# jizongFox/MI-based-Regularized-Semi-supervised-Segmentation

Hardware: AMD Instinct MI355X
Metric: images/sec (UNet+IIC fwd/bwd) ACDC 256^2 (higher is better)
Workload: dtype bf16; 1 GPU; udaiic train step, ACDC-shaped 1x256x256 4-class slices, LB=UB=16 per GPU, taps Conv5/Up_conv3/Up_conv2, K=20 x 5 sub-heads, paddings [1,3] (BASELINE configs[1]); mi_precision=f16f8, global_batch=32, parallelism=dp1, launch_tape=True, tape_ops=170, tape_replays_in_run=449

## Files before the change

mi-based-regularized-semi-supervised-segmentation_amd/csrc/api.hip:

```cpp
#include <stdarg.h>

#include "common.h"

namespace miseg_core {
static thread_local char g_err[512] = "";
char* last_error_buf() { return g_err; }
int fail(int code, const char* fmt, ...) {
    va_list ap;
    va_start(ap, fmt);
    vsnprintf(g_err, sizeof(g_err), fmt, ap);
    va_end(ap);
    return code;
}
}

extern "C" int miseg_version(void) { return 418; }
extern "C" const char* miseg_last_error(void) { return miseg::last_error_buf(); }

namespace miseg_core {
static hipEvent_t next_fork_event() {
    constexpr int kRing = 256, kDev = 16;
    struct Ring { hipEvent_t ev[kRing]; int made = 0, next = 0; };
    static thread_local Ring rings[kDev];
    int dev = 0;
    if (hipGetDevice(&dev) != hipSuccess || dev < 0 || dev >= kDev) return nullptr;
    Ring& r = rings[dev];
    constexpr unsigned flags = hipEventDisableTiming | hipEventDisableSystemFence;
    if (r.made < kRing) {
        if (hipEventCreateWithFlags(&r.ev[r.made], flags) != hipSuccess) return nullptr;
        ++r.made;
    }
    hipEvent_t ev = r.ev[r.next % r.made];
    r.next = (r.next + 1) % kRing;
    return ev;
}
}

extern "C" int miseg_stream_wait_stream(void* waiter, void* producer) {
    MISEG_TAPE(miseg_stream_wait_stream, waiter, producer);
    if (waiter == producer) return MISEG_OK;
    hipEvent_t ev = miseg_core::next_fork_event();
    if (!ev) return miseg_core::fail(MISEG_E_LAUNCH, "stream_wait_stream: hipEventCreateWithFlags failed");
    hipError_t e = hipEventRecord(ev, reinterpret_cast<hipStream_t>(producer));
    if (e == hipSuccess) e = hipStreamWaitEvent(reinterpret_cast<hipStream_t>(waiter), ev, 0);
    if (e != hipSuccess) return miseg_core::fail(MISEG_E_LAUNCH, "stream_wait_stream: %s", hipGetErrorString(e));
    return MISEG_OK;
}
```

mi-based-regularized-semi-supervised-segmentation_amd/csrc/conv_wgrad.hip:

```cpp
#include "conv.h"

namespace miseg {

constexpr int WG_TH = 8, WG_TW = 32, WG_P = 34;

template <typename T, bool BNL = false>
__global__ __launch_bounds__(kCT, 1) void conv3x3_wgrad_kernel(ConvSrc src, int N, int H, int W, const T* __restrict__ gout, int Cout,
                                                              int nsplit, float* __restrict__ partials, BnLoad bl) {
    extern __shared__ __attribute__((aligned(16))) float wsm[];
    float* Gs = wsm;
    float* Is = wsm + WG_TH * WG_TW * WG_P;
    const int Cin = src.C0 + src.C1;
    const int tid = threadIdx.x, lane = tid & 63, wv = tid >> 6, l15 = lane & 15, kq = lane >> 4;
    const int split = blockIdx.x, ci0 = blockIdx.y * 32, co0 = blockIdx.z * 32;
    const int tilesC = (W + WG_TW - 1) / WG_TW, tilesR = (H + WG_TH - 1) / WG_TH;
    const int ntiles = N * tilesR * tilesC;
    constexpr int IW = WG_TW + 2;
    f32x4 acc[2][18];
#pragma unroll
    for (int a = 0; a < 2; ++a)
#pragma unroll
        for (int b = 0; b < 18; ++b) acc[a][b] = f32x4{0.f, 0.f, 0.f, 0.f};
    float bc[kBwdCoefRows] = {0.f, 0.f, 0.f, 0.f, 0.f, 0.f};
    if (BNL && co0 + (tid & 31) < Cout)
#pragma unroll
        for (int r = 0; r < kBwdCoefRows; ++r) bc[r] = bl.coef[(size_t)r * Cout + co0 + (tid & 31)];

    for (int tile = split; tile < ntiles; tile += nsplit) {
        const int tc = tile % tilesC, tr = (tile / tilesC) % tilesR, n = tile / (tilesC * tilesR);
        const int h0 = tr * WG_TH, w0 = tc * WG_TW;
        __syncthreads();
        for (int idx = tid; idx < WG_TH * WG_TW * 32; idx += kCT) {
            const int c = idx & 31, px = idx >> 5, ix = px % WG_TW, iy = px / WG_TW;
            const int h = h0 + iy, w = w0 + ix;
            float v = 0.f;
            if (h < H && w < W && co0 + c < Cout) {
                const size_t o = (((size_t)n * H + h) * W + w) * Cout + co0 + c;
                v = to_f32(gout[o]);
                if (BNL) {
                    const float g = to_f32(reinterpret_cast<const T*>(bl.gy)[o]);
                    const float lin = bc[4] + bc[5] * (v - bc[2]);
                    v = v * bc[0] + bc[1] > relu_keep_threshold<T>() ? bc[3] * g + lin : lin;
                }
            }
            Gs[px * WG_P + c] = v;
        }
        for (int idx = tid; idx < (WG_TH + 2) * IW * 32; idx += kCT) {
            const int c = idx & 31, px = idx >> 5, ix = px % IW, iy = px / IW;
            const int h = h0 - 1 + iy, w = w0 - 1 + ix, cc = ci0 + c;
            float v = 0.f;
            if (h >= 0 && h < H && w >= 0 && w < W && cc < Cin) {
                if (cc < src.C0) {
                    const int hs = H >> src.ups0, wsz = W >> src.ups0;
                    v = to_f32(reinterpret_cast<const T*>(src.p0)[(((size_t)n * hs + (h >> src.ups0)) * wsz + (w >> src.ups0)) * src.C0 + cc]);
                } else {
                    const int hs = H >> src.ups1, wsz = W >> src.ups1;
                    v = to_f32(reinterpret_cast<const T*>(src.p1)[(((size_t)n * hs + (h >> src.ups1)) * wsz + (w >> src.ups1)) * src.C1 + cc - src.C0]);
                }
            }
            Is[px * WG_P + c] = v;
        }
        __syncthreads();
#pragma unroll 1
        for (int rr = 0; rr < 2; ++rr) {
            const int row = wv * 2 + rr;
#pragma unroll 1
            for (int cs = 0; cs < WG_TW; cs += 4) {
                const float a0 = Gs[(row * WG_TW + cs + kq) * WG_P + l15];
                const float a1 = Gs[(row * WG_TW + cs + kq) * WG_P + 16 + l15];
#pragma unroll
                for (int tap = 0; tap < 9; ++tap) {
                    const int ky = tap / 3, kx = tap % 3;
                    const float* ip = Is + ((row + ky) * IW + cs + kq + kx) * WG_P + l15;
                    const float b0 = ip[0], b1 = ip[16];
                    acc[0][tap * 2 + 0] = __builtin_amdgcn_mfma_f32_16x16x4f32(a0, b0, acc[0][tap * 2 + 0], 0, 0, 0);
                    acc[0][tap * 2 + 1] = __builtin_amdgcn_mfma_f32_16x16x4f32(a0, b1, acc[0][tap * 2 + 1], 0, 0, 0);
                    acc[1][tap * 2 + 0] = __builtin_amdgcn_mfma_f32_16x16x4f32(a1, b0, acc[1][tap * 2 + 0], 0, 0, 0);
                    acc[1][tap * 2 + 1] = __builtin_amdgcn_mfma_f32_16x16x4f32(a1, b1, acc[1][tap * 2 + 1], 0, 0, 0);
                }
            }
        }
    }
    float* Ds = wsm;
    for (int w = 0; w < 4; ++w) {
        __syncthreads();
        if (wv == w) {
#pragma unroll
            for (int a = 0; a < 2; ++a)
#pragma unroll
                for (int b = 0; b < 18; ++b)
#pragma unroll
                    for (int r = 0; r < 4; ++r) {
                        const int co = a * 16 + kq * 4 + r, col = (b / 2) * 32 + (b % 2) * 16 + l15;
                        if (w == 0) Ds[co * 288 + col] = acc[a][b][r];
                        else Ds[co * 288 + col] += acc[a][b][r];
                    }
        }
    }
    __syncthreads();
    float* outp = partials + (((size_t)split * gridDim.z + blockIdx.z) * gridDim.y + blockIdx.y) * (32 * 288);
    for (int e = tid; e < 32 * 288; e += kCT) outp[e] = Ds[e];
}

typedef __bf16 bf16x8_t __attribute__((ext_vector_type(8)));
typedef float f32x16 __attribute__((ext_vector_type(16)));
#define LDS_S16X4(ptr) ((__attribute__((address_space(3))) s16x4*)(ptr))

__device__ __forceinline__ bf16x8_t tr_frag32(const short* row_px0, int kq, int q, int p) {
    s16x4 lo = __builtin_amdgcn_ds_read_tr16_b64_v4i16(LDS_S16X4(row_px0 + (4 * kq + q) * 16 + 4 * p));
    s16x4 hi = __builtin_amdgcn_ds_read_tr16_b64_v4i16(LDS_S16X4(row_px0 + (16 + 4 * kq + q) * 16 + 4 * p));
    s16x8 f = {lo[0], lo[1], lo[2], lo[3], hi[0], hi[1], hi[2], hi[3]};
    return __builtin_bit_cast(bf16x8_t, f);
}

__device__ __forceinline__ bf16x8_t tr_frag(const short* blk_px0, int q, int p) {
    s16x4 lo = __builtin_amdgcn_ds_read_tr16_b64_v4i16(LDS_S16X4(blk_px0 + q * 16 + 4 * p));
    s16x4 hi = __builtin_amdgcn_ds_read_tr16_b64_v4i16(LDS_S16X4(blk_px0 + (4 + q) * 16 + 4 * p));
    s16x8 f = {lo[0], lo[1], lo[2], lo[3], hi[0], hi[1], hi[2], hi[3]};
    return __builtin_bit_cast(bf16x8_t, f);
}

template <bool BNL>
__global__ __launch_bounds__(kCT, 2) void conv3x3_wgrad_bf16_kernel(ConvSrc src, int N, int H, int W, const bf16* __restrict__ gout,
                                                                   int Cout, int nsplit, float* __restrict__ partials, BnLoad bl) {
    constexpr int IW = WG_TW + 2, NPX = WG_TH * WG_TW, NIPX = (WG_TH + 2) * IW;
    extern __shared__ __attribute__((aligned(16))) unsigned char wsm_raw[];
    constexpr int GSUB = NPX * 16 + 64;
    short* Gs = reinterpret_cast<short*>(wsm_raw);
    short* Is = Gs + 2 * GSUB;
    static_assert((NIPX * 32) % 256 == 128, "Is sub-tiles: re-check the bank offset for this tile shape");
    const int Cin = src.C0 + src.C1;
    const int tid = threadIdx.x, lane = tid & 63, wv = tid >> 6, l15 = lane & 15, kq = lane >> 4;
    const int g8 = 8 * kq, q = (lane >> 2) & 3, p4 = lane & 3;
    const int split = blockIdx.x, ci0 = blockIdx.y * 32, co0 = blockIdx.z * 32;
    const int tilesC = (W + WG_TW - 1) / WG_TW, tilesR = (H + WG_TH - 1) / WG_TH;
    const int ntiles = N * tilesR * tilesC;
    f32x16 acc[3];
#pragma unroll
    for (int b = 0; b < 3; ++b)
#pragma unroll
        for (int r = 0; r < 16; ++r) acc[b][r] = 0.f;
    const int wvu = __builtin_amdgcn_readfirstlane(wv);
    const int tap0 = 2 * wvu, tap1 = 2 * wvu + 1;
    const int off0 = ((tap0 / 3) * IW + tap0 % 3) * 16, off1 = ((tap1 / 3) * IW + tap1 % 3) * 16, off8 = (2 * IW + 2) * 16;
    const uint4 zero4 = make_uint4(0, 0, 0, 0);
    const int g16 = lane >> 4, chh = g16 & 1, pxh = g16 >> 1;

    constexpr int NG = NPX * 4 / kCT, NI = (NIPX * 4 + kCT - 1) / kCT;
    uint4 pg[NG], pi[NI];
    uint4 pr[BNL ? NG : 1];
    unsigned okg = 0;
    float* Cf = reinterpret_cast<float*>(Is + 2 * NIPX * 16);
    if (BNL) {
        for (int idx = tid; idx < kBwdCoefRows * 32; idx += kCT) Cf[idx] = co0 + (idx & 31) < Cout ? bl.coef[(size_t)(idx >> 5) * Cout + co0 + (idx & 31)] : 0.f;
        __syncthreads();
    }
    int g_iy[NG], g_ix[NG], g_rel[NG];
    int i_iy[NI], i_ix[NI], i_rel[NI], i_src[NI];
    {
        const int hs0 = H >> src.ups0, ws0 = W >> src.ups0, ws1 = W >> src.ups1;
        (void)hs0;
#pragma unroll
        for (int j = 0; j < NG; ++j) {
            const int idx = tid + kCT * j, v = idx & 3, px = idx >> 2, c = co0 + v * 8;
            g_ix[j] = px % WG_TW, g_iy[j] = px / WG_TW;
            g_rel[j] = c < Cout ? (g_iy[j] * W + g_ix[j]) * Cout + c : -1;
        }
#pragma unroll
        for (int j = 0; j < NI; ++j) {
            const int idx = tid + kCT * j, v = idx & 3, px = idx >> 2, cc = ci0 + v * 8;
            i_ix[j] = px % IW - 1, i_iy[j] = px / IW - 1;
            const bool slot = idx < NIPX * (3 + 1) && cc < Cin, first = cc < src.C0;
            i_src[j] = slot ? (first ? 0 : 1) : -1;
            i_rel[j] = first ? ((i_iy[j] >> src.ups0) * ws0 + (i_ix[j] >> src.ups0)) * src.C0 + cc
                             : ((i_iy[j] >> src.ups1) * ws1 + (i_ix[j] >> src.ups1)) * src.C1 + cc - src.C0;
        }
    }
    auto fetch = [&](int tile) __attribute__((always_inline)) {
        const int tc = tile % tilesC, tr = (tile / tilesC) % tilesR, n = tile / (tilesC * tilesR);
        const int h0 = tr * WG_TH, w0 = tc * WG_TW;
        const bf16* gcorner = gout + (((size_t)n * H + h0) * W + w0) * Cout;
        const bf16* ycorner = BNL ? reinterpret_cast<const bf16*>(bl.gy) + (((size_t)n * H + h0) * W + w0) * Cout : nullptr;
        const bf16* s0 = reinterpret_cast<const bf16*>(src.p0) + (((size_t)n * (H >> src.ups0) + (h0 >> src.ups0)) * (W >> src.ups0) + (w0 >> src.ups0)) * src.C0;
        const bf16* s1 = reinterpret_cast<const bf16*>(src.p1) + (((size_t)n * (H >> src.ups1) + (h0 >> src.ups1)) * (W >> src.ups1) + (w0 >> src.ups1)) * src.C1;
        okg = 0;
#pragma unroll
        for (int j = 0; j < NG; ++j) {
            uint4 val = zero4;
            if (g_rel[j] >= 0 && g_iy[j] < H - h0 && g_ix[j] < W - w0) {
                if (BNL) { pr[j] = *reinterpret_cast<const uint4*>(gcorner + g_rel[j]); val = *reinterpret_cast<const uint4*>(ycorner + g_rel[j]); okg |= 1u << j; }
                else val = *reinterpret_cast<const uint4*>(gcorner + g_rel[j]);
            }
            pg[j] = val;
        }
#pragma unroll
        for (int j = 0; j < NI; ++j) {
            uint4 val = zero4;
            if (i_src[j] >= 0 && (unsigned)(h0 + i_iy[j]) < (unsigned)H && (unsigned)(w0 + i_ix[j]) < (unsigned)W)
                val = *reinterpret_cast<const uint4*>((i_src[j] ? s1 : s0) + i_rel[j]);
            pi[j] = val;
        }
    };
    if (split < ntiles) fetch(split);
    for (int tile = split; tile < ntiles; tile += nsplit) {
        __syncthreads();
        if (BNL) {
            asm volatile("" ::: "memory");
            float cf[kBwdCoefRows][8];
#pragma unroll
            for (int r = 0; r < kBwdCoefRows; ++r)
#pragma unroll
                for (int i = 0; i < 8; i += 4) {
                    const float4 q = *reinterpret_cast<const float4*>(Cf + r * 32 + (tid & 3) * 8 + i);
                    cf[r][i] = q.x; cf[r][i + 1] = q.y; cf[r][i + 2] = q.z; cf[r][i + 3] = q.w;
                }
#pragma unroll
            for (int j = 0; j < NG; ++j)
                pg[j] = (okg >> j) & 1u ? bn_graw_vec<bf16>(pr[j], pg[j], cf[0], cf[1], cf[2], cf[3], cf[4], cf[5]) : zero4;
        }
#pragma unroll
        for (int j = 0; j < NG; ++j) {
            const int idx = tid + kCT * j, v = idx & 3, px = idx >> 2;
            *reinterpret_cast<uint4*>(Gs + (v >> 1) * GSUB + px * 16 + (v & 1) * 8) = pg[j];
        }
#pragma unroll
        for (int j = 0; j < NI; ++j) {
            const int idx = tid + kCT * j, v = idx & 3, px = idx >> 2;
            if (idx < NIPX * 4) *reinterpret_cast<uint4*>(Is + ((v >> 1) * NIPX + px) * 16 + (v & 1) * 8) = pi[j];
        }
        __syncthreads();
        if (tile + nsplit < ntiles) fetch(tile + nsplit);
#pragma unroll 2
        for (int row = 0; row < WG_TH; ++row) {
            const short* gb = Gs + chh * GSUB + (row * WG_TW + 8 * pxh) * 16;
            const bf16x8_t a0 = tr_frag(gb, q, p4), a1 = tr_frag(gb + 16 * 16, q, p4);
            const short* ib = Is + (chh * NIPX + row * IW + 8 * pxh) * 16;
            {
                const bf16x8_t b0 = tr_frag(ib + off0, q, p4), b1 = tr_frag(ib + off0 + 16 * 16, q, p4);
                acc[0] = __builtin_amdgcn_mfma_f32_32x32x16_bf16(a0, b0, acc[0], 0, 0, 0);
                acc[0] = __builtin_amdgcn_mfma_f32_32x32x16_bf16(a1, b1, acc[0], 0, 0, 0);
            }
            {
                const bf16x8_t b0 = tr_frag(ib + off1, q, p4), b1 = tr_frag(ib + off1 + 16 * 16, q, p4);
                acc[1] = __builtin_amdgcn_mfma_f32_32x32x16_bf16(a0, b0, acc[1], 0, 0, 0);
                acc[1] = __builtin_amdgcn_mfma_f32_32x32x16_bf16(a1, b1, acc[1], 0, 0, 0);
            }
            if ((row >> 1) == wvu) {
                const bf16x8_t b0 = tr_frag(ib + off8, q, p4), b1 = tr_frag(ib + off8 + 16 * 16, q, p4);
                acc[2] = __builtin_amdgcn_mfma_f32_32x32x16_bf16(a0, b0, acc[2], 0, 0, 0);
                acc[2] = __builtin_amdgcn_mfma_f32_32x32x16_bf16(a1, b1, acc[2], 0, 0, 0);
            }
        }
    }
    float* Ds = reinterpret_cast<float*>(wsm_raw);
    float* D8 = Ds + 32 * 288;
    __syncthreads();
#pragma unroll
    for (int r = 0; r < 16; ++r) {
        const int co = (r & 3) + 8 * (r >> 2) + 4 * (lane >> 5), ci = lane & 31;
        Ds[co * 288 + tap0 * 32 + ci] = acc[0][r];
        Ds[co * 288 + tap1 * 32 + ci] = acc[1][r];
        D8[wvu * 1024 + co * 32 + ci] = acc[2][r];
    }
    __syncthreads();
    float* outp = partials + (((size_t)split * gridDim.z + blockIdx.z) * gridDim.y + blockIdx.y) * (32 * 288);
    for (int e = tid; e < 32 * 288; e += kCT) {
        const int co = e / 288, col = e - co * 288;
        float v = Ds[e];
        if (col >= 256) {
            const int i8 = co * 32 + col - 256;
            v = (D8[i8] + D8[1024 + i8]) + (D8[2048 + i8] + D8[3072 + i8]);
        }
        outp[e] = v;
    }
}

template <bool BNL>
__global__ __launch_bounds__(kCT, BNL ? 3 : 4) void conv3x3_wgrad_bf16_c16_kernel(ConvSrc src, int N, int H, int W, const bf16* __restrict__ gout,
                                                                       int Cout, int nsplit, float* __restrict__ partials, BnLoad bl) {
    constexpr int IW = WG_TW + 2, NPX = WG_TH * WG_TW, NIPX = (WG_TH + 2) * IW;
    extern __shared__ __attribute__((aligned(16))) unsigned char wsm_raw[];
    short* Gs = reinterpret_cast<short*>(wsm_raw);
    short* Is = Gs + NPX * 16;
    const int Cin = src.C0 + src.C1;
    const int tid = threadIdx.x, lane = tid & 63, wv = tid >> 6, l15 = lane & 15, kq = lane >> 4;
    const int q = (lane >> 2) & 3, p4 = lane & 3;
    const int split = blockIdx.x, ci0 = blockIdx.y * 16, co0 = blockIdx.z * 16;
    const int tilesC = (W + WG_TW - 1) / WG_TW, tilesR = (H + WG_TH - 1) / WG_TH;
    const int ntiles = N * tilesR * tilesC;
    f32x4 acc[9];
#pragma unroll
    for (int b = 0; b < 9; ++b) acc[b] = f32x4{0.f, 0.f, 0.f, 0.f};
    const uint4 zero4 = make_uint4(0, 0, 0, 0);
    constexpr int NG = NPX * 2 / kCT, NI = (NIPX * 2 + kCT - 1) / kCT;
    uint4 pg[NG], pi[NI];
    uint4 pr[BNL ? NG : 1];
    unsigned okg = 0;
    float* Cf = reinterpret_cast<float*>(Is + NIPX * 16);
    if (BNL) {
        for (int idx = tid; idx < kBwdCoefRows * 16; idx += kCT) Cf[idx] = co0 + (idx & 15) < Cout ? bl.coef[(size_t)(idx >> 4) * Cout + co0 + (idx & 15)] : 0.f;
        __syncthreads();
    }
    int g_iy[NG], g_ix[NG], g_rel[NG];
    int i_iy[NI], i_ix[NI], i_rel[NI], i_src[NI];
    {
        const int hs0 = H >> src.ups0, ws0 = W >> src.ups0, ws1 = W >> src.ups1;
        (void)hs0;
#pragma unroll
        for (int j = 0; j < NG; ++j) {
            const int idx = tid + kCT * j, v = idx & 1, px = idx >> 1, c = co0 + v * 8;
            g_ix[j] = px % WG_TW, g_iy[j] = px / WG_TW;
            g_rel[j] = c < Cout ? (g_iy[j] * W + g_ix[j]) * Cout + c : -1;
        }
#pragma unroll
        for (int j = 0; j < NI; ++j) {
            const int idx = tid + kCT * j, v = idx & 1, px = idx >> 1, cc = ci0 + v * 8;
            i_ix[j] = px % IW - 1, i_iy[j] = px / IW - 1;
            const bool slot = idx < NIPX * (1 + 1) && cc < Cin, first = cc < src.C0;
            i_src[j] = slot ? (first ? 0 : 1) : -1;
            i_rel[j] = first ? ((i_iy[j] >> src.ups0) * ws0 + (i_ix[j] >> src.ups0)) * src.C0 + cc
                             : ((i_iy[j] >> src.ups1) * ws1 + (i_ix[j] >> src.ups1)) * src.C1 + cc - src.C0;
        }
    }
    auto fetch = [&](int tile) __attribute__((always_inline)) {
        const int tc = tile % tilesC, tr = (tile / tilesC) % tilesR, n = tile / (tilesC * tilesR);
        const int h0 = tr * WG_TH, w0 = tc * WG_TW;
        const bf16* gcorner = gout + (((size_t)n * H + h0) * W + w0) * Cout;
        const bf16* ycorner = BNL ? reinterpret_cast<const bf16*>(bl.gy) + (((size_t)n * H + h0) * W + w0) * Cout : nullptr;
        const bf16* s0 = reinterpret_cast<const bf16*>(src.p0) + (((size_t)n * (H >> src.ups0) + (h0 >> src.ups0)) * (W >> src.ups0) + (w0 >> src.ups0)) * src.C0;
        const bf16* s1 = reinterpret_cast<const bf16*>(src.p1) + (((size_t)n * (H >> src.ups1) + (h0 >> src.ups1)) * (W >> src.ups1) + (w0 >> src.ups1)) * src.C1;
        okg = 0;
#pragma unroll
        for (int j = 0; j < NG; ++j) {
            uint4 val = zero4;
            if (g_rel[j] >= 0 && g_iy[j] < H - h0 && g_ix[j] < W - w0) {
                if (BNL) { pr[j] = *reinterpret_cast<const uint4*>(gcorner + g_rel[j]); val = *reinterpret_cast<const uint4*>(ycorner + g_rel[j]); okg |= 1u << j; }
                else val = *reinterpret_cast<const uint4*>(gcorner + g_rel[j]);
            }
            pg[j] = val;
        }
#pragma unroll
        for (int j = 0; j < NI; ++j) {
            uint4 val = zero4;
            if (i_src[j] >= 0 && (unsigned)(h0 + i_iy[j]) < (unsigned)H && (unsigned)(w0 + i_ix[j]) < (unsigned)W)
                val = *reinterpret_cast<const uint4*>((i_src[j] ? s1 : s0) + i_rel[j]);
            pi[j] = val;
        }
    };
    if (split < ntiles) fetch(split);
    for (int tile = split; tile < ntiles; tile += nsplit) {
        __syncthreads();
        if (BNL) {
            asm volatile("" ::: "memory");
            float cf[kBwdCoefRows][8];
#pragma unroll
            for (int r = 0; r < kBwdCoefRows; ++r)
#pragma unroll
                for (int i = 0; i < 8; i += 4) {
                    const float4 q = *reinterpret_cast<const float4*>(Cf + r * 16 + (tid & 1) * 8 + i);
                    cf[r][i] = q.x; cf[r][i + 1] = q.y; cf[r][i + 2] = q.z; cf[r][i + 3] = q.w;
                }
#pragma unroll
            for (int j = 0; j < NG; ++j)
                pg[j] = (okg >> j) & 1u ? bn_graw_vec<bf16>(pr[j], pg[j], cf[0], cf[1], cf[2], cf[3], cf[4], cf[5]) : zero4;
        }
#pragma unroll
        for (int j = 0; j < NG; ++j) {
            const int idx = tid + kCT * j;
            *reinterpret_cast<uint4*>(Gs + (idx >> 1) * 16 + (idx & 1) * 8) = pg[j];
        }
#pragma unroll
        for (int j = 0; j < NI; ++j) {
            const int idx = tid + kCT * j;
            if (idx < NIPX * 2) *reinterpret_cast<uint4*>(Is + (idx >> 1) * 16 + (idx & 1) * 8) = pi[j];
        }
        __syncthreads();
        if (tile + nsplit < ntiles) fetch(tile + nsplit);
#pragma unroll
        for (int rr = 0; rr < 2; ++rr) {
            const int row = wv * 2 + rr;
            const bf16x8_t a0 = tr_frag32(Gs + row * WG_TW * 16, kq, q, p4);
#pragma unroll
            for (int tap = 0; tap < 9; ++tap) {
                const int ky = tap / 3, kx = tap % 3;
                const bf16x8_t b0 = tr_frag32(Is + ((row + ky) * IW + kx) * 16, kq, q, p4);
                acc[tap] = __builtin_amdgcn_mfma_f32_16x16x32_bf16(a0, b0, acc[tap], 0, 0, 0);
            }
        }
    }
    float* Ds = reinterpret_cast<float*>(wsm_raw);
    for (int w = 0; w < 4; ++w) {
        __syncthreads();
        if (wv == w) {
#pragma unroll
            for (int tap = 0; tap < 9; ++tap)
#pragma unroll
                for (int r = 0; r < 4; ++r) {
                    const int o = (kq * 4 + r) * 144 + tap * 16 + l15;
                    if (w == 0) Ds[o] = acc[tap][r];
                    else Ds[o] += acc[tap][r];
                }
        }
    }
    __syncthreads();
    const int nci32 = (Cin + 31) / 32, nco32 = (Cout + 31) / 32;
    float* outp = partials + (((size_t)split * nco32 + blockIdx.z / 2) * nci32 + blockIdx.y / 2) * (32 * 288) + (blockIdx.y & 1) * 16;
    for (int e = tid; e < 16 * 144; e += kCT) {
        const int co = (blockIdx.z & 1) * 16 + e / 144, tap = (e % 144) / 16, ci = e % 16;
        outp[co * 288 + tap * 32 + ci] = Ds[e];
    }
}

__global__ __launch_bounds__(256) void wgrad_reduce_kernel(const float* __restrict__ partials, int nsplit, int Cout, int Cin, int nco,
                                                           int nci, float* __restrict__ gw) {
    const size_t stride = (size_t)nco * nci * (32 * 288);
    reduce_partials_block(partials, nsplit, stride, nco * nci * 32 * 288, gw, [](int e) { return (size_t)e; }, [=](int e) {
        const int ci32 = e & 31, tap = (e >> 5) % 9, co32 = (e / 288) & 31, tile = e / (32 * 288);
        const int co = (tile / nci) * 32 + co32, ci = (tile % nci) * 32 + ci32;
        return (co < Cout && ci < Cin) ? (co * Cin + ci) * 9 + tap : -1;
    });
}

}

using namespace miseg;

namespace miseg {
__global__ __launch_bounds__(256) void slice_cin_kernel(const float* __restrict__ src, int Cout, int Cin_pad, int Cin, float* __restrict__ dst) {
    const int total = Cout * Cin * 9;
    for (int e = blockIdx.x * 256 + threadIdx.x; e < total; e += gridDim.x * 256) {
        const int t = e % 9, ci = (e / 9) % Cin, co = e / (9 * Cin);
        dst[e] = src[((size_t)co * Cin_pad + ci) * 9 + t];
    }
}
}
extern "C" int miseg_conv3x3_wgrad_slice(void* stream, const float* gw_padded, int64_t Cout, int64_t Cin_pad, int64_t Cin, float* gw) {
    MISEG_TAPE(miseg_conv3x3_wgrad_slice, stream, gw_padded, Cout, Cin_pad, Cin, gw);
    MISEG_REQUIRE(gw_padded && gw && Cout > 0 && Cin > 0 && Cin <= Cin_pad, "conv3x3_wgrad_slice: bad args");
    const int total = (int)(Cout * Cin * 9);
    hipLaunchKernelGGL(slice_cin_kernel, dim3(std::min((total + 255) / 256, 256)), dim3(256), 0, as_stream(stream), gw_padded, (int)Cout, (int)Cin_pad,
                       (int)Cin, gw);
    MISEG_LAUNCH_CHECK("slice_cin_kernel");
    return MISEG_OK;
}

static int wgrad_splits(int64_t N, int64_t H, int64_t W, int64_t Cin, int64_t Cout) {
    const int64_t ntiles = N * cdiv(H, WG_TH) * cdiv(W, WG_TW);
    const int64_t per = cdiv(Cin, 32) * cdiv(Cout, 32);
    static const int target = [] { const char* e = getenv("MISEG_WGRAD_BLOCKS"); return e ? atoi(e) : 256; }();
    int64_t s = std::max<int64_t>(1, target / per);
    return (int)std::min<int64_t>(s, ntiles);
}

extern "C" int64_t miseg_conv3x3_wgrad_ws_bytes(int64_t N, int64_t H, int64_t W, int64_t Cin, int64_t Cout) {
    return (int64_t)wgrad_splits(N, H, W, Cin, Cout) * cdiv(Cin, 32) * cdiv(Cout, 32) * 32 * 288 * 4;
}

static int conv3x3_wgrad_impl(void* stream, int dt, const void* in0, int64_t C0, int ups0, const void* in1, int64_t C1, int ups1, int64_t N,
                              int64_t H, int64_t W, const void* gout, int64_t Cout, float* gw, void* ws, int64_t ws_bytes, BnLoad bl) {
    MISEG_REQUIRE(in0 && gout && gw && ws, "conv3x3_wgrad: null pointer");
    MISEG_REQUIRE(C1 == 0 || in1, "conv3x3_wgrad: second source missing");
    const int64_t Cin = C0 + C1;
    MISEG_REQUIRE(ws_bytes >= miseg_conv3x3_wgrad_ws_bytes(N, H, W, Cin, Cout), "conv3x3_wgrad: workspace too small");
    ConvSrc s{in0, in1, (int)C0, (int)C1, ups0, ups1};
    const int ns = wgrad_splits(N, H, W, Cin, Cout), nci = (int)cdiv(Cin, 32), nco = (int)cdiv(Cout, 32);
    const size_t lb = ((size_t)WG_TH * WG_TW + (WG_TH + 2) * (WG_TW + 2)) * WG_P * 4;
    hipStream_t st = as_stream(stream);
    dim3 grid(ns, nci, nco);
    MISEG_WITH_STORAGE_TYPE(dt, "conv3x3_wgrad",
    if constexpr (std::is_same_v<TT, float>) {
        if (bl.gy) {
            hipFuncSetAttribute((const void*)conv3x3_wgrad_kernel<TT, true>, hipFuncAttributeMaxDynamicSharedMemorySize, (int)lb);
            hipLaunchKernelGGL((conv3x3_wgrad_kernel<TT, true>), grid, dim3(kCT), lb, st, s, (int)N, (int)H, (int)W, (const TT*)gout, (int)Cout, ns, (float*)ws, bl);
        } else {
            hipFuncSetAttribute((const void*)conv3x3_wgrad_kernel<TT, false>, hipFuncAttributeMaxDynamicSharedMemorySize, (int)lb);
            hipLaunchKernelGGL((conv3x3_wgrad_kernel<TT, false>), grid, dim3(kCT), lb, st, s, (int)N, (int)H, (int)W, (const TT*)gout, (int)Cout, ns, (float*)ws, bl);
        }
    } else {
        MISEG_REQUIRE(C0 % 8 == 0 && C1 % 8 == 0 && Cout % 8 == 0, "conv3x3_wgrad: bf16 needs channel counts that are multiples of 8");
        const size_t lbb = std::max<size_t>(((size_t)2 * WG_TH * WG_TW + 2 * (WG_TH + 2) * (WG_TW + 2)) * 16 * 2 + 2 * 64 * 2, (size_t)(32 * 288 + 4 * 1024) * 4);
        const bool narrow = Cout % 16 == 0 && (std::min(Cin, Cout) <= 16 || (Cin == 32 && Cout == 64));
        if (narrow || Cout <= 16) {
            const size_t lbc = (size_t)(WG_TH * WG_TW + (WG_TH + 2) * (WG_TW + 2)) * 16 * 2 + (bl.gy ? kBwdCoefRows * 16 * 4 : 0);
            dim3 gridc(ns, (unsigned)cdiv(Cin, 16), (unsigned)cdiv(Cout, 16));
            if (bl.gy) hipLaunchKernelGGL(conv3x3_wgrad_bf16_c16_kernel<true>, gridc, dim3(kCT), lbc, st, s, (int)N, (int)H, (int)W, (const bf16*)gout, (int)Cout, ns, (float*)ws, bl);
            else hipLaunchKernelGGL(conv3x3_wgrad_bf16_c16_kernel<false>, gridc, dim3(kCT), lbc, st, s, (int)N, (int)H, (int)W, (const bf16*)gout, (int)Cout, ns, (float*)ws, bl);
        } else if (bl.gy) {
            hipFuncSetAttribute((const void*)conv3x3_wgrad_bf16_kernel<true>, hipFuncAttributeMaxDynamicSharedMemorySize, (int)lbb);
            hipLaunchKernelGGL(conv3x3_wgrad_bf16_kernel<true>, grid, dim3(kCT), lbb, st, s, (int)N, (int)H, (int)W, (const bf16*)gout, (int)Cout, ns, (float*)ws, bl);
        } else {
            hipFuncSetAttribute((const void*)conv3x3_wgrad_bf16_kernel<false>, hipFuncAttributeMaxDynamicSharedMemorySize, (int)lbb);
            hipLaunchKernelGGL(conv3x3_wgrad_bf16_kernel<false>, grid, dim3(kCT), lbb, st, s, (int)N, (int)H, (int)W, (const bf16*)gout, (int)Cout, ns, (float*)ws, bl);
        }
    }
    return MISEG_OK);
    MISEG_LAUNCH_CHECK("conv3x3_wgrad_kernel");
    const int total = nco * nci * 32 * 288;
    hipLaunchKernelGGL(wgrad_reduce_kernel, dim3(reduce_grid(total, ns)), dim3(256), 0, st, (const float*)ws, ns, (int)Cout, (int)Cin, nco, nci, gw);
    MISEG_LAUNCH_CHECK("wgrad_reduce_kernel");
    return MISEG_OK;
}

extern "C" int miseg_conv3x3_wgrad(void* stream, int dt, const void* in0, int64_t C0, int ups0, const void* in1, int64_t C1, int ups1,
                                   int64_t N, int64_t H, int64_t W, const void* gout, int64_t Cout, float* gw, void* ws, int64_t ws_bytes) {
    MISEG_TAPE(miseg_conv3x3_wgrad, stream, dt, in0, C0, ups0, in1, C1, ups1, N, H, W, gout, Cout, gw, ws, ws_bytes);
    MISEG_F16_DISPATCH_ON(dt, miseg_conv3x3_wgrad, stream, MISEG_BF16, in0, C0, ups0, in1, C1, ups1, N, H, W, gout, Cout, gw, ws, ws_bytes);
    return conv3x3_wgrad_impl(stream, dt, in0, C0, ups0, in1, C1, ups1, N, H, W, gout, Cout, gw, ws, ws_bytes, BnLoad{nullptr, nullptr});
}

extern "C" int miseg_conv3x3_wgrad_bn(void* stream, int dt, const void* in0, int64_t C0, int ups0, const void* in1, int64_t C1, int ups1,
                                      int64_t N, int64_t H, int64_t W, const void* raw, const void* gy, const float* bwd_coef, int64_t Cout,
                                      float* gw, void* ws, int64_t ws_bytes) {
    MISEG_TAPE(miseg_conv3x3_wgrad_bn, stream, dt, in0, C0, ups0, in1, C1, ups1, N, H, W, raw, gy, bwd_coef, Cout, gw, ws, ws_bytes);
    MISEG_F16_DISPATCH_ON(dt, miseg_conv3x3_wgrad_bn, stream, MISEG_BF16, in0, C0, ups0, in1, C1, ups1, N, H, W, raw, gy, bwd_coef, Cout, gw, ws, ws_bytes);
    MISEG_REQUIRE(gy && bwd_coef, "conv3x3_wgrad_bn: null pointer");
    MISEG_REQUIRE(Cout % (dt == MISEG_F32 ? 4 : 8) == 0, "conv3x3_wgrad_bn: Cout must be a whole number of 16-byte vectors");
    return conv3x3_wgrad_impl(stream, dt, in0, C0, ups0, in1, C1, ups1, N, H, W, raw, Cout, gw, ws, ws_bytes, BnLoad{gy, bwd_coef});
}
```

Measured before the change: 4948 images/s.

## Restructure narrow bf16 wgrad kernel: two Cin slices per block, buffer loads, tap-split waves

The narrow-channel bf16 weight-gradient kernel now handles up to two 16-channel input slices per block (NSL template), so each loaded output-gradient tile is reused across 32 input channels and the grid y-dimension halves. Global loads move to raw buffer loads with an out-of-range offset sentinel, replacing per-slot bounds branches and precomputed index arrays. MFMA work is split by tap across waves instead of by rows, which cuts per-thread accumulators and changes the final shared-memory reduction. The trade-off is more register pressure from doubled prefetch buffers, extra barriers per slice, and more complex indexing. A profiling script for wgrad kernel times is also added.

```diff
diff --git a/mi-based-regularized-semi-supervised-segmentation_amd/csrc/api.hip b/mi-based-regularized-semi-supervised-segmentation_amd/csrc/api.hip
--- a/mi-based-regularized-semi-supervised-segmentation_amd/csrc/api.hip
+++ b/mi-based-regularized-semi-supervised-segmentation_amd/csrc/api.hip
@@ -14,7 +14,7 @@
 }
 }
 
-extern "C" int miseg_version(void) { return 418; }
+extern "C" int miseg_version(void) { return 419; }
 extern "C" const char* miseg_last_error(void) { return miseg::last_error_buf(); }
 
 namespace miseg_core {
diff --git a/mi-based-regularized-semi-supervised-segmentation_amd/csrc/conv_wgrad.hip b/mi-based-regularized-semi-supervised-segmentation_amd/csrc/conv_wgrad.hip
--- a/mi-based-regularized-semi-supervised-segmentation_amd/csrc/conv_wgrad.hip
+++ b/mi-based-regularized-semi-supervised-segmentation_amd/csrc/conv_wgrad.hip
@@ -275,7 +275,15 @@
     }
 }
 
-template <bool BNL>
+constexpr unsigned kWgOOB = 0xFFFFFF00u;
+__device__ __forceinline__ __amdgpu_buffer_rsrc_t wg_rsrc(const void* p, long long byte_off) {
+    return __builtin_amdgcn_make_buffer_rsrc((void*)((const char*)p + byte_off), 0, 0x7FFFFFFF, 0x00020000);
+}
+__device__ __forceinline__ uint4 wg_ld16(__amdgpu_buffer_rsrc_t r, unsigned off) {
+    return __builtin_bit_cast(uint4, __builtin_amdgcn_raw_buffer_load_b128(r, (int)off, 0, 0));
+}
+
+template <bool BNL, int NSL>
 __global__ __launch_bounds__(kCT, BNL ? 3 : 4) void conv3x3_wgrad_bf16_c16_kernel(ConvSrc src, int N, int H, int W, const bf16* __restrict__ gout,
                                                                        int Cout, int nsplit, float* __restrict__ partials, BnLoad bl) {
     constexpr int IW = WG_TW + 2, NPX = WG_TH * WG_TW, NIPX = (WG_TH + 2) * IW;
@@ -285,15 +293,19 @@
     const int Cin = src.C0 + src.C1;
     const int tid = threadIdx.x, lane = tid & 63, wv = tid >> 6, l15 = lane & 15, kq = lane >> 4;
     const int q = (lane >> 2) & 3, p4 = lane & 3;
-    const int split = blockIdx.x, ci0 = blockIdx.y * 16, co0 = blockIdx.z * 16;
+    const int wvu = __builtin_amdgcn_readfirstlane(wv);
+    const int split = blockIdx.x, ci0 = blockIdx.y * (16 * NSL), co0 = blockIdx.z * 16;
     const int tilesC = (W + WG_TW - 1) / WG_TW, tilesR = (H + WG_TH - 1) / WG_TH;
     const int ntiles = N * tilesR * tilesC;
-    f32x4 acc[9];
-#pragma unroll
-    for (int b = 0; b < 9; ++b) acc[b] = f32x4{0.f, 0.f, 0.f, 0.f};
+    f32x4 acc[NSL][3];
+#pragma unroll
+    for (int s = 0; s < NSL; ++s)
+#pragma unroll
+        for (int b = 0; b < 3; ++b) acc[s][b] = f32x4{0.f, 0.f, 0.f, 0.f};
     const uint4 zero4 = make_uint4(0, 0, 0, 0);
     constexpr int NG = NPX * 2 / kCT, NI = (NIPX * 2 + kCT - 1) / kCT;
-    uint4 pg[NG], pi[NI];
+    static_assert(kCT == 256 && WG_TW == 32 && WG_TH == 8, "the slot geometry and the tap split below are written for 256 threads and 8 x 32 tiles");
+    uint4 pg[NG], pi[NSL][NI];
     uint4 pr[BNL ? NG : 1];
     unsigned okg = 0;
     float* Cf = reinterpret_cast<float*>(Is + NIPX * 16);
@@ -301,112 +313,138 @@
         for (int idx = tid; idx < kBwdCoefRows * 16; idx += kCT) Cf[idx] = co0 + (idx & 15) < Cout ? bl.coef[(size_t)(idx >> 4) * Cout + co0 + (idx & 15)] : 0.f;
         __syncthreads();
     }
-    int g_iy[NG], g_ix[NG], g_rel[NG];
-    int i_iy[NI], i_ix[NI], i_rel[NI], i_src[NI];
-    {
-        const int hs0 = H >> src.ups0, ws0 = W >> src.ups0, ws1 = W >> src.ups1;
-        (void)hs0;
-#pragma unroll
-        for (int j = 0; j < NG; ++j) {
-            const int idx = tid + kCT * j, v = idx & 1, px = idx >> 1, c = co0 + v * 8;
-            g_ix[j] = px % WG_TW, g_iy[j] = px / WG_TW;
-            g_rel[j] = c < Cout ? (g_iy[j] * W + g_ix[j]) * Cout + c : -1;
-        }
-#pragma unroll
-        for (int j = 0; j < NI; ++j) {
-            const int idx = tid + kCT * j, v = idx & 1, px = idx >> 1, cc = ci0 + v * 8;
-            i_ix[j] = px % IW - 1, i_iy[j] = px / IW - 1;
-            const bool slot = idx < NIPX * (1 + 1) && cc < Cin, first = cc < src.C0;
-            i_src[j] = slot ? (first ? 0 : 1) : -1;
-            i_rel[j] = first ? ((i_iy[j] >> src.ups0) * ws0 + (i_ix[j] >> src.ups0)) * src.C0 + cc
-                             : ((i_iy[j] >> src.ups1) * ws1 + (i_ix[j] >> src.ups1)) * src.C1 + cc - src.C0;
-        }
-    }
-    auto fetch = [&](int tile) __attribute__((always_inline)) {
+    const int v8 = (tid & 1) * 8;
+    const int g_ix = (tid >> 1) & 31, g_iy = tid >> 6;
+    const bool g_ch = co0 + v8 < Cout;
+    const unsigned g_off = ((g_iy * W + g_ix) * Cout + co0 + v8) * 2u, g_step = 4u * W * Cout * 2u;
+    unsigned i_yx[NI], i_off[NSL][NI];
+#pragma unroll
+    for (int j = 0; j < NI; ++j) {
+        const int px = (tid + kCT * j) >> 1, ix = px % IW - 1, iy = px / IW - 1;
+        i_yx[j] = (iy + 1) | (ix + 1) << 8;
+#pragma unroll
+        for (int s = 0; s < NSL; ++s) {
+            const int cc = ci0 + 16 * s + v8;
+            const int e = cc < src.C0 ? (((iy >> src.ups0) + 1) * (W >> src.ups0) + (ix >> src.ups0) + 1) * src.C0 + cc
+                                      : (((iy >> src.ups1) + 1) * (W >> src.ups1) + (ix >> src.ups1) + 1) * src.C1 + cc - src.C0;
+            i_off[s][j] = px < NIPX && cc < Cin ? (unsigned)e * 2u : kWgOOB;
+        }
+    }
+    auto fetch_g = [&](int tile) __attribute__((always_inline)) {
         const int tc = tile % tilesC, tr = (tile / tilesC) % tilesR, n = tile / (tilesC * tilesR);
         const int h0 = tr * WG_TH, w0 = tc * WG_TW;
-        const bf16* gcorner = gout + (((size_t)n * H + h0) * W + w0) * Cout;
-        const bf16* ycorner = BNL ? reinterpret_cast<const bf16*>(bl.gy) + (((size_t)n * H + h0) * W + w0) * Cout : nullptr;
-        const bf16* s0 = reinterpret_cast<const bf16*>(src.p0) + (((size_t)n * (H >> src.ups0) + (h0 >> src.ups0)) * (W >> src.ups0) + (w0 >> src.ups0)) * src.C0;
-        const bf16* s1 = reinterpret_cast<const bf16*>(src.p1) + (((size_t)n * (H >> src.ups1) + (h0 >> src.ups1)) * (W >> src.ups1) + (w0 >> src.ups1)) * src.C1;
+        const long long corner = ((((long long)n * H + h0) * W + w0) * Cout) * 2;
+        const __amdgpu_buffer_rsrc_t rg = wg_rsrc(gout, corner);
+        const __amdgpu_buffer_rsrc_t ry = wg_rsrc(BNL ? bl.gy : gout, corner);
         okg = 0;
 #pragma unroll
         for (int j = 0; j < NG; ++j) {
-            uint4 val = zero4;
-            if (g_rel[j] >= 0 && g_iy[j] < H - h0 && g_ix[j] < W - w0) {
-                if (BNL) { pr[j] = *reinterpret_cast<const uint4*>(gcorner + g_rel[j]); val = *reinterpret_cast<const uint4*>(ycorner + g_rel[j]); okg |= 1u << j; }
-                else val = *reinterpret_cast<const uint4*>(gcorner + g_rel[j]);
-            }
-            pg[j] = val;
-        }
+            const bool in = g_ch && g_iy + 4 * j < H - h0 && g_ix < W - w0;
+            const unsigned off = in ? g_off + j * g_step : kWgOOB;
+            if (BNL) { pr[j] = wg_ld16(rg, off); pg[j] = wg_ld16(ry, off); okg |= in ? 1u << j : 0u; }
+            else pg[j] = wg_ld16(rg, off);
+        }
+    };
+    auto fetch_i = [&](int tile, int s) __attribute__((always_inline)) {
+        const int tc = tile % tilesC, tr = (tile / tilesC) % tilesR, n = tile / (tilesC * tilesR);
+        const int h0 = tr * WG_TH, w0 = tc * WG_TW;
+        const int ws0 = W >> src.ups0, ws1 = W >> src.ups1;
+        const __amdgpu_buffer_rsrc_t r0 = wg_rsrc(src.p0, ((((long long)n * (H >> src.ups0) + (h0 >> src.ups0) - 1) * ws0 + (w0 >> src.ups0) - 1) * src.C0) * 2);
+        const __amdgpu_buffer_rsrc_t r1 = wg_rsrc(src.p1, ((((long long)n * (H >> src.ups1) + (h0 >> src.ups1) - 1) * ws1 + (w0 >> src.ups1) - 1) * src.C1) * 2);
+        const bool lo0 = ci0 + 16 * s < src.C0, hi0 = ci0 + 16 * s + 8 < src.C0;
 #pragma unroll
         for (int j = 0; j < NI; ++j) {
-            uint4 val = zero4;
-            if (i_src[j] >= 0 && (unsigned)(h0 + i_iy[j]) < (unsigned)H && (unsigned)(w0 + i_ix[j]) < (unsigned)W)
-                val = *reinterpret_cast<const uint4*>((i_src[j] ? s1 : s0) + i_rel[j]);
-            pi[j] = val;
+            const bool in = h0 - 1 + (i_yx[j] & 0xff) < (unsigned)H && w0 - 1 + (i_yx[j] >> 8) < (unsigned)W;
+            const unsigned off = in ? i_off[s][j] : kWgOOB;
+            if (lo0 == hi0) pi[s][j] = wg_ld16(lo0 ? r0 : r1, off);
+            else {
+                const uint4 a = wg_ld16(r0, v8 ? kWgOOB : off), b = wg_ld16(r1, v8 ? off : kWgOOB);
+                pi[s][j] = make_uint4(a.x | b.x, a.y | b.y, a.z | b.z, a.w | b.w);
+            }
         }
     };
-    if (split < ntiles) fetch(split);
+    if (split < ntiles) {
+        fetch_g(split);
+#pragma unroll
+        for (int s = 0; s < NSL; ++s) fetch_i(split, s);
+    }
+    const int t0 = 2 * wvu, t1 = 2 * wvu + 1;
+    const int off0 = ((t0 / 3) * IW + t0 % 3) * 16, off1 = ((t1 / 3) * IW + t1 % 3) * 16, off8 = (2 * IW + 2) * 16;
     for (int tile = split; tile < ntiles; tile += nsplit) {
-        __syncthreads();
-        if (BNL) {
-            asm volatile("" ::: "memory");
-            float cf[kBwdCoefRows][8];
-#pragma unroll
-            for (int r = 0; r < kBwdCoefRows; ++r)
-#pragma unroll
-                for (int i = 0; i < 8; i += 4) {
-                    const float4 q = *reinterpret_cast<const float4*>(Cf + r * 16 + (tid & 1) * 8 + i);
-                    cf[r][i] = q.x; cf[r][i + 1] = q.y; cf[r][i + 2] = q.z; cf[r][i + 3] = q.w;
-                }
-#pragma unroll
-            for (int j = 0; j < NG; ++j)
-                pg[j] = (okg >> j) & 1u ? bn_graw_vec<bf16>(pr[j], pg[j], cf[0], cf[1], cf[2], cf[3], cf[4], cf[5]) : zero4;
-        }
-#pragma unroll
-        for (int j = 0; j < NG; ++j) {
-            const int idx = tid + kCT * j;
-            *reinterpret_cast<uint4*>(Gs + (idx >> 1) * 16 + (idx & 1) * 8) = pg[j];
-        }
-#pragma unroll
-        for (int j = 0; j < NI; ++j) {
-            const int idx = tid + kCT * j;
-            if (idx < NIPX * 2) *reinterpret_cast<uint4*>(Is + (idx >> 1) * 16 + (idx & 1) * 8) = pi[j];
-        }
-        __syncthreads();
-        if (tile + nsplit < ntiles) fetch(tile + nsplit);
-#pragma unroll
-        for (int rr = 0; rr < 2; ++rr) {
-            const int row = wv * 2 + rr;
-            const bf16x8_t a0 = tr_frag32(Gs + row * WG_TW * 16, kq, q, p4);
-#pragma unroll
-            for (int tap = 0; tap < 9; ++tap) {
-                const int ky = tap / 3, kx = tap % 3;
-                const bf16x8_t b0 = tr_frag32(Is + ((row + ky) * IW + kx) * 16, kq, q, p4);
-                acc[tap] = __builtin_amdgcn_mfma_f32_16x16x32_bf16(a0, b0, acc[tap], 0, 0, 0);
-            }
-        }
-    }
+        const bool more = tile + nsplit < ntiles;
+#pragma unroll
+        for (int s = 0; s < NSL; ++s) {
+            __syncthreads();
+            if (s == 0) {
+                if (BNL) {
+                    asm volatile("" ::: "memory");
+                    float cf[kBwdCoefRows][8];
+#pragma unroll
+                    for (int r = 0; r < kBwdCoefRows; ++r)
+#pragma unroll
+                        for (int i = 0; i < 8; i += 4) {
+                            const float4 c4 = *reinterpret_cast<const float4*>(Cf + r * 16 + v8 + i);
+                            cf[r][i] = c4.x; cf[r][i + 1] = c4.y; cf[r][i + 2] = c4.z; cf[r][i + 3] = c4.w;
+                        }
+#pragma unroll
+                    for (int j = 0; j < NG; ++j)
+                        pg[j] = (okg >> j) & 1u ? bn_graw_vec<bf16>(pr[j], pg[j], cf[0], cf[1], cf[2], cf[3], cf[4], cf[5]) : zero4;
+                }
+#pragma unroll
+                for (int j = 0; j < NG; ++j) {
+                    const int idx = tid + kCT * j;
+                    *reinterpret_cast<uint4*>(Gs + (idx >> 1) * 16 + (idx & 1) * 8) = pg[j];
+                }
+            }
+#pragma unroll
+            for (int j = 0; j < NI; ++j) {
+                const int idx = tid + kCT * j;
+                if (idx < NIPX * 2) *reinterpret_cast<uint4*>(Is + (idx >> 1) * 16 + (idx & 1) * 8) = pi[s][j];
+            }
+            __syncthreads();
+            if (more) {
+                if (s == 0) fetch_g(tile + nsplit);
+                fetch_i(tile + nsplit, s);
+            }
+#pragma unroll
+            for (int row = 0; row < WG_TH; ++row) {
+                const bf16x8_t a0 = tr_frag32(Gs + row * WG_TW * 16, kq, q, p4);
+                const short* ib = Is + row * IW * 16;
+                acc[s][0] = __builtin_amdgcn_mfma_f32_16x16x32_bf16(a0, tr_frag32(ib + off0, kq, q, p4), acc[s][0], 0, 0, 0);
+                acc[s][1] = __builtin_amdgcn_mfma_f32_16x16x32_bf16(a0, tr_frag32(ib + off1, kq, q, p4), acc[s][1], 0, 0, 0);
+                if ((row >> 1) == wvu) acc[s][2] = __builtin_amdgcn_mfma_f32_16x16x32_bf16(a0, tr_frag32(ib + off8, kq, q, p4), acc[s][2], 0, 0, 0);
+            }
+        }
+    }
+    constexpr int DW = 9 * 16 * NSL;
     float* Ds = reinterpret_cast<float*>(wsm_raw);
+    static_assert(16 * DW * 4 <= (NPX + NIPX) * 32, "the reduced tile must fit in the operand tiles");
+    __syncthreads();
+#pragma unroll
+    for (int s = 0; s < NSL; ++s)
+#pragma unroll
+        for (int r = 0; r < 4; ++r) {
+            Ds[(kq * 4 + r) * DW + (t0 * NSL + s) * 16 + l15] = acc[s][0][r];
+            Ds[(kq * 4 + r) * DW + (t1 * NSL + s) * 16 + l15] = acc[s][1][r];
+        }
     for (int w = 0; w < 4; ++w) {
-        __syncthreads();
-        if (wv == w) {
-#pragma unroll
-            for (int tap = 0; tap < 9; ++tap)
+        if (w) __syncthreads();
+        if (wvu == w) {
+#pragma unroll
+            for (int s = 0; s < NSL; ++s)
 #pragma unroll
                 for (int r = 0; r < 4; ++r) {
-                    const int o = (kq * 4 + r) * 144 + tap * 16 + l15;
-                    if (w == 0) Ds[o] = acc[tap][r];
-                    else Ds[o] += acc[tap][r];
+                    const int o = (kq * 4 + r) * DW + (8 * NSL + s) * 16 + l15;
+                    if (w == 0) Ds[o] = acc[s][2][r];
+                    else Ds[o] += acc[s][2][r];
                 }
         }
     }
     __syncthreads();
     const int nci32 = (Cin + 31) / 32, nco32 = (Cout + 31) / 32;
-    float* outp = partials + (((size_t)split * nco32 + blockIdx.z / 2) * nci32 + blockIdx.y / 2) * (32 * 288) + (blockIdx.y & 1) * 16;
-    for (int e = tid; e < 16 * 144; e += kCT) {
-        const int co = (blockIdx.z & 1) * 16 + e / 144, tap = (e % 144) / 16, ci = e % 16;
+    float* outp = partials + (((size_t)split * nco32 + blockIdx.z / 2) * nci32 + blockIdx.y) * (32 * 288);
+    for (int e = tid; e < 16 * DW; e += kCT) {
+        const int co = (blockIdx.z & 1) * 16 + e / DW, col = e % DW, tap = col / (16 * NSL), ci = col % (16 * NSL);
         outp[co * 288 + tap * 32 + ci] = Ds[e];
     }
 }
@@ -482,9 +520,14 @@
         const bool narrow = Cout % 16 == 0 && (std::min(Cin, Cout) <= 16 || (Cin == 32 && Cout == 64));
         if (narrow || Cout <= 16) {
             const size_t lbc = (size_t)(WG_TH * WG_TW + (WG_TH + 2) * (WG_TW + 2)) * 16 * 2 + (bl.gy ? kBwdCoefRows * 16 * 4 : 0);
-            dim3 gridc(ns, (unsigned)cdiv(Cin, 16), (unsigned)cdiv(Cout, 16));
-            if (bl.gy) hipLaunchKernelGGL(conv3x3_wgrad_bf16_c16_kernel<true>, gridc, dim3(kCT), lbc, st, s, (int)N, (int)H, (int)W, (const bf16*)gout, (int)Cout, ns, (float*)ws, bl);
-            else hipLaunchKernelGGL(conv3x3_wgrad_bf16_c16_kernel<false>, gridc, dim3(kCT), lbc, st, s, (int)N, (int)H, (int)W, (const bf16*)gout, (int)Cout, ns, (float*)ws, bl);
+            dim3 gridc(ns, (unsigned)nci, (unsigned)cdiv(Cout, 16));
+            if (Cin <= 16) {
+                if (bl.gy) hipLaunchKernelGGL((conv3x3_wgrad_bf16_c16_kernel<true, 1>), gridc, dim3(kCT), lbc, st, s, (int)N, (int)H, (int)W, (const bf16*)gout, (int)Cout, ns, (float*)ws, bl);
+                else hipLaunchKernelGGL((conv3x3_wgrad_bf16_c16_kernel<false, 1>), gridc, dim3(kCT), lbc, st, s, (int)N, (int)H, (int)W, (const bf16*)gout, (int)Cout, ns, (float*)ws, bl);
+            } else {
+                if (bl.gy) hipLaunchKernelGGL((conv3x3_wgrad_bf16_c16_kernel<true, 2>), gridc, dim3(kCT), lbc, st, s, (int)N, (int)H, (int)W, (const bf16*)gout, (int)Cout, ns, (float*)ws, bl);
+                else hipLaunchKernelGGL((conv3x3_wgrad_bf16_c16_kernel<false, 2>), gridc, dim3(kCT), lbc, st, s, (int)N, (int)H, (int)W, (const bf16*)gout, (int)Cout, ns, (float*)ws, bl);
+            }
         } else if (bl.gy) {
             hipFuncSetAttribute((const void*)conv3x3_wgrad_bf16_kernel<true>, hipFuncAttributeMaxDynamicSharedMemorySize, (int)lbb);
             hipLaunchKernelGGL(conv3x3_wgrad_bf16_kernel<true>, grid, dim3(kCT), lbb, st, s, (int)N, (int)H, (int)W, (const bf16*)gout, (int)Cout, ns, (float*)ws, bl);
diff --git a/profiles/wgrad_kernel_times.py b/profiles/wgrad_kernel_times.py
--- /dev/null
+++ b/profiles/wgrad_kernel_times.py
@@ -0,0 +1,22 @@
+import csv, sys, collections
+rows = list(csv.DictReader(open(sys.argv[1])))
+ev = sorted((int(r["Start_Timestamp"]), int(r["End_Timestamp"]), r["Kernel_Name"], r["Stream_Id"], r.get("Grid_Size_X", r.get("Grid_Size", "")), r.get("Grid_Size_Y", ""), r.get("Grid_Size_Z", "")) for r in rows)
+adam = [i for i, e in enumerate(ev) if "adam" in e[2]]
+steps = [ev[adam[i - 1] + 1:adam[i] + 1] for i in range(max(1, len(adam) - 6), len(adam))]
+def fam(n):
+    for k in ("conv3x3_wgrad_bf16_c16", "conv3x3_wgrad_bf16_kernel", "wgrad_reduce", "stem_wgrad_kernel", "stem_wgrad_sum", "bn_relu_bwd_reduce", "bn_bwd_apply"):
+        if k in n: return k
+    return None
+tot = collections.defaultdict(float); cnt = collections.defaultdict(int)
+for g in steps:
+    for s, e, n, st, *_ in g:
+        f = fam(n)
+        if f: tot[f] += e - s; cnt[f] += 1
+ns = len(steps)
+for f in tot: print(f"{f}: {tot[f]/ns/1e3:.1f} us/step, {cnt[f]/ns:.1f} calls/step, avg {tot[f]/cnt[f]/1e3:.1f} us")
+w = sum(tot[f] for f in tot if "wgrad" in f)
+print(f"wgrad family total {w/ns/1e3:.1f} us/step over {ns} steps; step lengths us:", [round((max(e[1] for e in g) - g[0][0]) / 1e3) for g in steps])
+steps.sort(key=lambda g: max(e[1] for e in g) - g[0][0]); g = steps[len(steps) // 2]; t0 = g[0][0]
+for s, e, n, st, gx, gy, gz in g:
+    if "conv3x3_wgrad" in n:
+        print(f"  {(s-t0)/1e3:8.1f} {(e-s)/1e3:7.1f} grid {gx} {gy} {gz} {'c16' if 'c16' in n else 'wide'}{n[n.find('<'):n.find('>')+1]}")
```

Measured after the change: 4921 images/s. No clear change (-0.5%).
